# RobustFieldAutonomyLab/Distributional_RL_Navigation

Measured on AMD Instinct MI355X. Metric: env steps/sec (whole node) at 65 536 envs; IQN grad-steps/sec, higher is better.
Workload: dtype f32; 1 GPU; 65536 envs/GPU + IQN training (act K=32, 8 quantiles, replay 100000, batch 256, 1 grad step(s) every 4 vector steps); envs_per_gpu=65536, n_cores=8, n_obstacles=10, precision=f64, learner=independent, ranks_per_gpu=1, act_variant=2, taus=per_env, resets=under_next_act, launches_per_grad_step=1, ablation=False

## Files before the change

distributional_rl_navigation_amd/csrc/mn_capi.hip:

```cpp
#include <math.h>
#include <stdio.h>
#include <stdlib.h>
#include <string.h>

#include <string>
#include <vector>

#include "mn_internal.h"

struct mn_handle {
    MnArrays A;
    MnDev P;
    mn_params params;
    std::vector<void *> allocs;
    std::string err;
    int step_parity = 0;
    int last_parity = 0;
    uint32_t *seeds_dev = nullptr;
    uint32_t *mask_count = nullptr;
    int32_t *list_scratch = nullptr;
    double *peek_scratch = nullptr;
    double *obs64_buf = nullptr, *rew64_buf = nullptr;
    double *traj_trace = nullptr;
    int32_t traj_trace_steps = 0, traj_trace_sub = 0;
// ... 59 lines not shown
        snprintf(b, sizeof(b), "handle lives on HIP device %d but the calling thread's current device is %d", h->device, cur);
        return fail(h, MN_ERR_INVALID, b);
    }
    if (h->reset_pending) {
        if (hipEventSynchronize(h->ev_reset_end) != hipSuccess) return fail(h, MN_ERR_HIP, "waiting for the asynchronous reset failed");
        h->reset_pending = false;
    }
    if (h->reset_owed) {
        const hipStream_t s = h->owed_stream;
        settle_owed(h, s);
        if (hipStreamSynchronize(s) != hipSuccess) return fail(h, MN_ERR_HIP, "waiting for the owed reset failed");
    }
    return MN_OK;
}
static void join_reset(mn_handle *h, hipStream_t s) {
    if (!h) return;
    if (h->reset_owed) {
        int cur = -1;
        if (hipGetDevice(&cur) == hipSuccess && cur == h->device) settle_owed(h, s);
    }
    if (h->reset_pending) {
        if (hipStreamWaitEvent(s, h->ev_reset_end, 0) == hipSuccess) h->reset_pending = false;
    }
}
#define MN_ON_DEVICE(h) do { int _rc = on_device(h); if (_rc) return _rc; } while (0)

extern "C" int mn_default_params(mn_params *p) {
    if (!p) return MN_ERR_INVALID;
    memset(p, 0, sizeof(*p));
    p->width = 50; p->height = 50; p->core_r = 0.5; p->v_rel_max = 1.0; p->p = 0.8;
    p->v_range[0] = 5; p->v_range[1] = 10; p->obs_r_range[0] = 1; p->obs_r_range[1] = 3;
    p->clear_r = 10.0; p->goal_dis = 2.0; p->timestep_penalty = -1.0; p->collision_penalty = -50.0;
    p->goal_reward = 100.0; p->discount = 0.99; p->min_start_goal_dis = 25.0;
    p->init_theta = M_PI / 4; p->init_speed = 0.0;
    p->dt = 0.1; p->robot_r = 0.8; p->max_speed = 2.0;
    p->a[0] = -0.4; p->a[1] = 0.0; p->a[2] = 0.4;
    p->w[0] = -M_PI / 6; p->w[1] = 0.0; p->w[2] = M_PI / 6;
    p->sonar_range = 10.0; p->sonar_angle = 2 * M_PI / 3;
    p->num_cores = 8; p->num_obs = 5; p->reset_start_and_goal = 1; p->random_reset_state = 1;
    p->set_boundary = 0; p->max_episode_steps = 1000; p->N = 10; p->num_beams = MN_NUM_BEAMS;
    p->precision = MN_PRECISION_MIXED;
    return MN_OK;
}

static int derive(mn_handle *h, const mn_params &p) {
    const int32_t keep_skip = h->P.debug_skip;
    if (p.num_beams != MN_NUM_BEAMS) return fail(h, MN_ERR_INVALID, "num_beams must be 11");
    if (p.num_cores < 0 || p.num_cores > MN_MAX_CORES) return fail(h, MN_ERR_INVALID, "num_cores out of [0, 8]");
    if (p.num_obs < 0 || p.num_obs > MN_MAX_OBS) return fail(h, MN_ERR_INVALID, "num_obs out of [0, 10]");
    if (p.N < 1 || p.N > 1000) return fail(h, MN_ERR_INVALID, "robot N out of range");
    if (p.precision != MN_PRECISION_F64 && p.precision != MN_PRECISION_MIXED) return fail(h, MN_ERR_INVALID, "bad precision");
    if (p.step_lanes != 0 && p.step_lanes != 1 && p.step_lanes != 2 && p.step_lanes != 4 && p.step_lanes != 8) return fail(h, MN_ERR_INVALID, "step_lanes must be 0 (default), 1, 2, 4 or 8");
    if (p.rollout_lanes != 0 && p.rollout_lanes != 2 && p.rollout_lanes != 4 && p.rollout_lanes != 8 && p.rollout_lanes != 16) return fail(h, MN_ERR_INVALID, "rollout_lanes must be 0 (default), 2, 4, 8 or 16");
    MnDev &d = h->P;
    const int32_t keep_n = d.n_stages;
    d.width = p.width; d.height = p.height; d.core_r = p.core_r; d.v_rel_max = p.v_rel_max; d.p = p.p;
    d.v_lo = p.v_range[0]; d.v_span = p.v_range[1] - p.v_range[0];
    d.or_lo = p.obs_r_range[0]; d.or_span = p.obs_r_range[1] - p.obs_r_range[0];
    d.clear_r = p.clear_r; d.goal_dis = p.goal_dis;
    d.timestep_penalty = p.timestep_penalty; d.collision_penalty = p.collision_penalty; d.goal_reward = p.goal_reward;
    d.min_start_goal_dis = p.min_start_goal_dis; d.init_theta = p.init_theta; d.init_speed = p.init_speed;
    d.dt = p.dt; d.robot_r = p.robot_r; d.max_speed = p.max_speed;
    double amax = p.a[0];
    for (int i = 0; i < 3; ++i) {
        d.a[i] = p.a[i]; d.w[i] = p.w[i]; if (p.a[i] > amax) amax = p.a[i];
        d.rot_c[i] = cos(p.w[i] * p.dt); d.rot_s[i] = sin(p.w[i] * p.dt);
    }
    d.k_drag = amax / p.max_speed;
    d.sonar_range = p.sonar_range;
    const double phi = p.sonar_angle / (p.num_beams - 1);
    const double a0 = -p.sonar_angle / 2;
    for (int i = 0; i < MN_NUM_BEAMS; ++i) {
        d.beam_rel[i] = a0 + i * phi;
        d.beam_cos[i] = cos(d.beam_rel[i]);
        d.beam_sin[i] = sin(d.beam_rel[i]);
    }
    d.fan_sin = sin(p.sonar_angle / 2); d.fan_cos = cos(p.sonar_angle / 2);
    d.fan_filter = (p.sonar_angle / 2 < 0.49 * M_PI) ? 1 : 0;
    d.two_pi = 2 * M_PI;
    d.two_pi_r = 2 * M_PI * p.core_r;
    d.two_pi_vrel = 2 * M_PI * p.v_rel_max;
    d.inv_two_pi_vrel = 1.0 / d.two_pi_vrel;
    d.two_pi_r_r = 2 * M_PI * p.core_r * p.core_r;
    d.binom_q = exp(1.0 * log(1.0 - 0.5));
    d.sg_lo_x = 2.0; d.sg_span_x = (p.width - 2.0) - 2.0; d.sg_lo_y = 2.0; d.sg_span_y = (p.height - 2.0) - 2.0;
    d.c_span_x = p.width - 0.0; d.c_span_y = p.height - 0.0;
    d.o_lo = 5.0; d.o_span_x = (p.width - 5.0) - 5.0; d.o_span_y = (p.height - 5.0) - 5.0;
    d.num_cores = p.num_cores; d.num_obs = p.num_obs; d.reset_start_and_goal = p.reset_start_and_goal;
    d.random_reset_state = p.random_reset_state; d.set_boundary = p.set_boundary;
    d.max_episode_steps = p.max_episode_steps; d.N = p.N;
    d.n_stages = keep_n;
    d.debug_skip = keep_skip;
    h->params = p;
    return MN_OK;
}

template <typename T>
static int dev_alloc(mn_handle *h, T **out, size_t count, bool zero = true) {
    void *p = nullptr;
    hipError_t e = hipMalloc(&p, count * sizeof(T));
    if (e != hipSuccess) { h->err = std::string("hipMalloc failed: ") + hipGetErrorString(e); return MN_ERR_ALLOC; }
    if (zero) { e = hipMemset(p, 0, count * sizeof(T)); if (e != hipSuccess) { h->err = hipGetErrorString(e); return MN_ERR_HIP; } }
    h->allocs.push_back(p);
    *out = (T *)p;
    return MN_OK;
}

extern "C" int mn_destroy(mn_handle *h) {
    if (!h) return MN_ERR_INVALID;
    int cur = -1;
    const bool moved = hipGetDevice(&cur) == hipSuccess && h->device >= 0 && cur != h->device;
    if (moved) (void)hipSetDevice(h->device);
    if (h->reset_owed) { const hipStream_t s = h->owed_stream; settle_owed(h, s); (void)hipStreamSynchronize(s); }
    for (hipEvent_t e : h->ev) (void)hipEventDestroy(e);
    for (hipEvent_t e : h->ev_reset) (void)hipEventDestroy(e);
    if (h->side) { (void)hipStreamSynchronize(h->side); (void)hipStreamDestroy(h->side); }
    if (h->ev_stepped) (void)hipEventDestroy(h->ev_stepped);
    if (h->ev_reset_end) (void)hipEventDestroy(h->ev_reset_end);
    if (h->seen_host) (void)hipHostFree((void *)h->seen_host);
    for (void *p : h->allocs) (void)hipFree(p);
    if (moved) (void)hipSetDevice(cur);
    delete h;
    return MN_OK;
}

extern "C" int mn_create(int32_t n_envs, const mn_params *p, mn_handle **out) {
    if (!out || !p || n_envs <= 0) return fail(nullptr, MN_ERR_INVALID, "mn_create: bad arguments");
    int ndev = 0;
    if (hipGetDeviceCount(&ndev) != hipSuccess || ndev == 0) return fail(nullptr, MN_ERR_NO_DEVICE, "no HIP device visible");
    mn_handle *h = new mn_handle();
    if (hipGetDevice(&h->device) != hipSuccess) { delete h; return fail(nullptr, MN_ERR_HIP, "hipGetDevice failed"); }
    memset(&h->A, 0, sizeof(h->A));
    memset(&h->P, 0, sizeof(h->P));
    h->P.timestep_scale = 1.0;
    h->params.precision = p->precision;
    int rc = derive(h, *p);
    if (rc) { g_create_err = h->err; delete h; return rc; }
    MnArrays &A = h->A;
    A.n = n_envs;
    A.npad = (n_envs + MN_PAD - 1) / MN_PAD * MN_PAD;
    const size_t np = (size_t)A.npad;
#define ALLOC(field, count)                                    \
    if ((rc = dev_alloc(h, &A.field, (count))) != MN_OK) {      \
        g_create_err = h->err;                                 \
        mn_destroy(h);                                         \
        return rc;                                             \
    }
    ALLOC(x, np) ALLOC(y, np) ALLOC(theta, np) ALLOC(speed, np) ALLOC(vx, np) ALLOC(vy, np)
    ALLOC(start_x, np) ALLOC(start_y, np) ALLOC(goal_x, np) ALLOC(goal_y, np) ALLOC(init_theta, np) ALLOC(init_speed, np)
    ALLOC(ep_t, np) ALLOC(tot_t, np) ALLOC(counts, np)
    ALLOC(cx, np * MN_MAX_CORES) ALLOC(cy, np * MN_MAX_CORES) ALLOC(cg, np * MN_MAX_CORES)
    ALLOC(ox, np * MN_MAX_OBS) ALLOC(oy, np * MN_MAX_OBS) ALLOC(orad, np * MN_MAX_OBS)
    ALLOC(qcx, np * MN_MAX_CORES) ALLOC(qcy, np * MN_MAX_CORES) ALLOC(qcg, np * MN_MAX_CORES)
    ALLOC(qox, np * MN_MAX_OBS) ALLOC(qoy, np * MN_MAX_OBS) ALLOC(qor, np * MN_MAX_OBS)
    ALLOC(mt, np * 624) ALLOC(mt_pos, np)
    A.qcap = (int32_t)(((np >> 6) + MN_QSHARDS - 1) / MN_QSHARDS * 64);
    ALLOC(queue_count, 2 * MN_QWORDS) ALLOC(queue, (size_t)MN_QSHARDS * A.qcap)
#undef ALLOC
    if ((rc = dev_alloc(h, &h->seeds_dev, np)) || (rc = dev_alloc(h, &h->mask_count, 1)) ||
        (rc = dev_alloc(h, &h->list_scratch, np)) || (rc = dev_alloc(h, &h->peek_scratch, np))) {
        g_create_err = h->err; mn_destroy(h); return rc;
    }
    {
        std::vector<double> v(np);
        for (size_t i = 0; i < np; ++i) v[i] = 5.0;
        (void)hipMemcpy(A.start_x, v.data(), np * 8, hipMemcpyHostToDevice);
// ... 917 lines not shown
```

distributional_rl_navigation_amd/csrc/mn_internal.h:

```cpp
#pragma once
#include <hip/hip_runtime.h>
#include <stdint.h>

#include "marinenav_hip.h"

#define MN_WAVE 64
#define MN_PAD 256
#define MN_FIX_SCALE 16777216.0
#define MN_FIX_INV (1.0 / 16777216.0)
#define MN_TAB_ROWS (3 * MN_MAX_CORES + 3 * MN_MAX_OBS)

struct MnArrays {
    int32_t n, npad;
    double *x, *y, *theta, *speed, *vx, *vy;
    double *start_x, *start_y, *goal_x, *goal_y, *init_theta, *init_speed;
    int32_t *ep_t;
    int64_t *tot_t;
    int32_t *counts;
    double *cx, *cy, *cg;
    double *ox, *oy, *orad;
    int32_t *qcx, *qcy, *qox, *qoy;
    float *qcg, *qor;
    uint32_t *mt;
    int32_t *mt_pos;
    double *obs64;
    double *rew64;
    double *traj;
    int32_t traj_n;
    uint32_t *queue_count;
    int32_t *queue;
    int32_t qcap;
};
#define MN_QSHARDS 32
#define MN_QSTRIDE 32
#define MN_QWORDS (MN_QSHARDS * MN_QSTRIDE)

struct MnDev {
    double width, height, core_r, v_rel_max, p, v_lo, v_span, or_lo, or_span, clear_r, goal_dis;
    double timestep_penalty, collision_penalty, goal_reward;
    double min_start_goal_dis, init_theta, init_speed;
    double dt, robot_r, max_speed, k_drag, a[3], w[3];
    double sonar_range;
    double beam_rel[MN_NUM_BEAMS], beam_cos[MN_NUM_BEAMS], beam_sin[MN_NUM_BEAMS];
    double rot_c[3], rot_s[3];
    double fan_sin, fan_cos;
    int32_t fan_filter;
    double two_pi;
    double two_pi_r;
    double two_pi_vrel;
    double inv_two_pi_vrel;
    double two_pi_r_r;
    double binom_q;
    double sg_lo_x, sg_span_x, sg_lo_y, sg_span_y;
    double c_span_x, c_span_y;
    double o_lo, o_span_x, o_span_y;
    double timestep_scale;
    int32_t num_cores, num_obs, reset_start_and_goal, random_reset_state, set_boundary, max_episode_steps, N;
    int32_t n_stages;
    int32_t debug_skip;
    int64_t sched_t[MN_MAX_STAGES];
    int32_t sched_nc[MN_MAX_STAGES], sched_no[MN_MAX_STAGES];
    double sched_md[MN_MAX_STAGES];
};

struct MnRing {
    const float *prev_obs;
    float *states, *next_states;
    int64_t *actions;
    float *rewards, *dones;
    int64_t ptr, cap;
};

#define MN_STATE_MAGIC 0x54534e4du
#define MN_STATE_VERSION 1
#define MN_STATE_HEADER_BYTES 1024
#define MN_STATE_F64_ROWS (12 + 3 * MN_MAX_CORES + 3 * MN_MAX_OBS + 1)
#define MN_STATE_I32_ROWS (3 + 3 * MN_MAX_CORES + 3 * MN_MAX_OBS)
#define MN_STATE_MT_WORDS 624
struct MnStateHeader {
    uint32_t magic, version;
    int32_t n, precision;
    int64_t bytes;
    int32_t header_bytes, qcap;
    mn_params params;
    int32_t n_stages, pad0;
    double timestep_scale;
    int64_t sched_t[MN_MAX_STAGES];
    int32_t sched_nc[MN_MAX_STAGES], sched_no[MN_MAX_STAGES];
    double sched_md[MN_MAX_STAGES];
    int32_t step_parity, last_parity;
    uint32_t tick;
    int32_t under_act_max, owed_max_rows;
    uint32_t has_peak;
    uint32_t peak, seen;
};
static_assert(sizeof(MnStateHeader) <= MN_STATE_HEADER_BYTES, "MnStateHeader outgrew its slot");
static inline int64_t mn_state_layout_bytes(int64_t n, int64_t qcap) {
    return MN_STATE_HEADER_BYTES + n * MN_STATE_MT_WORDS * 4 + 2 * MN_QWORDS * 4 + MN_QSHARDS * qcap * 4 + MN_STATE_F64_ROWS * n * 8 + MN_STATE_I32_ROWS * n * 4;
}
void mn_launch_state(bool save, const MnArrays &A, const MnStateHeader &hdr, void *blob, uint32_t *peak_dev, uint32_t *seen_dev, uint32_t *ready, hipStream_t s);

void mn_launch_step(const MnArrays &A, const MnDev &P, int precision, int lanes, const int32_t *actions, float *obs,
                    float *reward, uint8_t *done, uint8_t *info, int parity, const MnRing *ring, hipStream_t s);
void mn_launch_rollout(const MnArrays &A, const MnDev &P, int precision, int lanes, int n_steps, const int32_t *actions_in,
                       uint64_t seed, uint64_t step0, uint64_t env0, float *obs_out, float *obs_trace, float *reward_trace,
                       uint8_t *done_trace, uint8_t *info_trace, int32_t *action_trace, hipStream_t s);
void mn_launch_random_actions(uint64_t seed, uint64_t step, uint64_t env0, int n, int32_t *out, hipStream_t s);
void mn_launch_rollout_policy(const MnArrays &A, const MnDev &P, int precision, int n_steps, int policy, float *obs_io, float *obs_trace,
                              float *reward_trace, uint8_t *done_trace, uint8_t *info_trace, int32_t *action_trace, double *traj_trace, hipStream_t s);
void mn_launch_planner_act(const float *obs, int n, int policy, const double *a, const double *w, int32_t *actions, hipStream_t s);
void mn_launch_rollout_iqn_rows(const MnArrays &A, const MnDev &P, int precision, int n_steps, const uint32_t *image, uint64_t *rng_state, float cvar,
                                int adaptive, const float *cvar_row, const uint8_t *adaptive_row, float *obs_io, float *obs_trace, float *reward_trace,
                                uint8_t *done_trace, uint8_t *info_trace, int32_t *action_trace, float *cvar_trace, float *q_trace, double *traj_trace,
                                uint32_t *words, int32_t *steps_run, hipStream_t s);
void mn_launch_rollout_iqn_eval(const MnArrays &A, const MnDev &P, int precision, int n_steps, const uint32_t *image, uint64_t *rng_state, float cvar,
                                int adaptive, const float *cvar_row, const uint8_t *adaptive_row, float *obs_io, float *obs_trace, float *reward_trace,
                                uint8_t *done_trace, uint8_t *info_trace, int32_t *action_trace, float *cvar_trace, float *q_trace, double *traj_trace,
                                float *quantiles_trace, float *taus_trace, uint32_t *words, int32_t *steps_run, hipStream_t s);
void mn_launch_rollout_iqn_groups(const MnArrays &A, const MnDev &P, int precision, int n_steps, const uint32_t *images, int64_t image_stride,
                                  int rows_per_group, uint64_t *rng_states, const float *cvar_row, const uint8_t *adaptive_row, float *obs_io,
                                  float *obs_trace, float *reward_trace, uint8_t *done_trace, uint8_t *info_trace, int32_t *action_trace, float *cvar_trace,
                                  float *q_trace, uint32_t *group_words, int32_t *steps_run, hipStream_t s);
int mn_iqn_rollout_image(mn_iqn_ctx *c, const float *const *weights, hipStream_t s, const uint32_t **image, uint32_t **words);
void mn_launch_dqn_pack(const float *const *weights, float *image_dev, hipStream_t s);
void mn_launch_rollout_dqn(const MnArrays &A, const MnDev &P, int precision, int n_steps, const float *image, float *obs_io, float *obs_trace,
                           float *reward_trace, uint8_t *done_trace, uint8_t *info_trace, int32_t *action_trace, float *q_trace, double *traj_trace, hipStream_t s);
void mn_launch_rollout_dqn_groups(const MnArrays &A, const MnDev &P, int precision, int n_steps, const float *images, int64_t image_stride, int n_groups,
                                  int rows_per_group, float *obs_io, float *obs_trace, float *reward_trace, uint8_t *done_trace, uint8_t *info_trace,
                                  int32_t *action_trace, float *q_trace, hipStream_t s);
void mn_launch_reset_under_act(const MnArrays &A, const MnDev &P, int precision, const uint32_t *count_dev, const int32_t *list_dev, float *obs,
                               uint32_t *ready, uint32_t tick, uint32_t *peak_dev, uint32_t *peak_host, hipStream_t s);
void mn_launch_reset(const MnArrays &A, const MnDev &P, int precision, const uint32_t *count_dev, uint32_t count_host,
                     const int32_t *list_dev, int mode, float *obs, hipStream_t s, uint32_t *peak_dev = nullptr, uint32_t *peak_host = nullptr, bool sharded = false);
#define MN_PREP_RESET_MIN_BLOCKS 256
// ... 39 lines not shown
```

distributional_rl_navigation_amd/csrc/mn_reset_body.h:

```cpp
#pragma once
#include "mn_device.h"

#ifdef MN_ABLATION
#define MN_RSKIP(bit) ((P.debug_skip & (bit)) != 0)
#else
#define MN_RSKIP(bit) false
#endif

#define MT_N 624
#define MT_M 397

__device__ __forceinline__ uint32_t mt_temper(uint32_t y) {
    y ^= (y >> 11);
    y ^= (y << 7) & 0x9d2c5680u;
    y ^= (y << 15) & 0xefc60000u;
    y ^= (y >> 18);
    return y;
}

__device__ __forceinline__ uint32_t mt_twist(uint32_t cur, uint32_t nxt, uint32_t far) {
    const uint32_t y = (cur & 0x80000000u) | (nxt & 0x7fffffffu);
    return far ^ (y >> 1) ^ ((y & 1u) ? 0x9908b0dfu : 0u);
}

// ... 377 lines not shown
                    }
                    for (int i = 0; i < no && valid; ++i) {
                        const double dx = W.ox[i] - x, dy = W.oy[i] - y;
                        valid = !dist_le(dx * dx + dy * dy, W.orad[i] + r);
                    }
                }
                int used = nb;
                for (;;) {
                    const unsigned long long m = __ballot(valid);
                    if (!m) break;
                    const int j = first_lane(m);
                    const double xj = bcast(x, j), yj = bcast(y, j), rj = bcast(r, j);
                    if (lane == j) { W.ox[no] = x; W.oy[no] = y; W.orad[no] = r; valid = false; }
                    else if (valid && lane > j) {
                        const double dx = xj - x, dy = yj - y;
                        valid = !dist_le(dx * dx + dy * dy, rj + r);
                    }
                    ++no;
                    if (no == want_o) { used = j + 1; break; }
                }
                __syncthreads();
                tried += used;
                rng.advance(6 * used);
                if (no == want_o || tried >= 500) break;
            }
        }

        if (P.random_reset_state) {
            rng.ensure(4, lane);
            double u[2];
            rng.template fetch<2>(0, u);
            th0 = 0.0 + (P.two_pi - 0.0) * u[0];
            sp0 = 0.0 + (P.max_speed - 0.0) * u[1];
            rng.advance(4);
        } else {
            th0 = P.init_theta; sp0 = P.init_speed;
        }

        __syncthreads();
        rng.store(A, e, lane, MN_RSKIP(512));
        if (lane < MN_MAX_CORES) {
            const bool v = lane < nc;
            A.cx[lane * np + e] = v ? W.cx[lane] : 0.0;
            A.cy[lane * np + e] = v ? W.cy[lane] : 0.0;
            A.cg[lane * np + e] = v ? W.cg[lane] : 0.0;
        }
        if (lane < MN_MAX_OBS) {
            const bool v = lane < no;
            A.ox[lane * np + e] = v ? W.ox[lane] : 0.0;
            A.oy[lane * np + e] = v ? W.oy[lane] : 0.0;
            A.orad[lane * np + e] = v ? W.orad[lane] : 0.0;
        }
        if (lane == 0) {
            A.mt_pos[e] = rng.c.pos;
            A.counts[e] = nc | (no << 8);
            A.start_x[e] = sx; A.start_y[e] = sy; A.goal_x[e] = gx; A.goal_y[e] = gy;
            A.init_theta[e] = th0; A.init_speed[e] = sp0;
        }
    } else {
        const int cnt = A.counts[e];
        nc = cnt & 0xff; no = (cnt >> 8) & 0xff;
        if (lane < nc) { W.cx[lane] = A.cx[lane * np + e]; W.cy[lane] = A.cy[lane * np + e]; W.cg[lane] = A.cg[lane * np + e]; }
        if (lane < no) { W.ox[lane] = A.ox[lane * np + e]; W.oy[lane] = A.oy[lane * np + e]; W.orad[lane] = A.orad[lane * np + e]; }
        sx = A.start_x[e]; sy = A.start_y[e]; gx = A.goal_x[e]; gy = A.goal_y[e];
        th0 = A.init_theta[e]; sp0 = A.init_speed[e];
    }
    __syncthreads();

    if (lane < MN_MAX_CORES) {
        const bool v = lane < nc;
        A.qcx[lane * np + e] = v ? __double2int_rn(W.cx[lane] * MN_FIX_SCALE) : 0;
        A.qcy[lane * np + e] = v ? __double2int_rn(W.cy[lane] * MN_FIX_SCALE) : 0;
        A.qcg[lane * np + e] = v ? (float)W.cg[lane] : 0.0f;
    }
    if (lane < MN_MAX_OBS) {
        const bool v = lane < no;
        A.qox[lane * np + e] = v ? __double2int_rn(W.ox[lane] * MN_FIX_SCALE) : 0;
        A.qoy[lane * np + e] = v ? __double2int_rn(W.oy[lane] * MN_FIX_SCALE) : 0;
        A.qor[lane * np + e] = v ? (float)W.orad[lane] : 0.0f;
    }

    double cvx = 0.0, cvy = 0.0;
    {
        const double i1 = 1.0 / P.two_pi_r_r, i2 = 1.0 / P.two_pi;
        for (int k = 0; k < nc; ++k) {
            double ux, uy;
            mn_core_velocity<double, true>(W.cx[k] - sx, W.cy[k] - sy, W.cg[k], i1, i2, ux, uy);
            cvx += ux; cvy += uy;
        }
    }
    double sn, cs;
    sincos(th0, &sn, &cs);
    const double velx = sp0 * cs + cvx, vely = sp0 * sn + cvy;

    if (lane < MN_NUM_BEAMS) {
        const double angle = th0 + P.beam_rel[lane];
        const bool up = fabs(angle - 0.5 * 3.141592653589793) < 1e-03;
        const bool down = fabs(angle - 3 * 3.141592653589793 / 2) < 1e-03;
        double bx = P.beam_cos[lane], by = P.beam_sin[lane];
        if (up || down) {
            const double sg = up ? 1.0 : -1.0;
            bx = sg * sn; by = sg * cs;
        }
        MnBeam<M> beam;
        beam.init();
        for (int k = 0; k < (MN_RSKIP(256) ? 0 : no); ++k) {
            const double mx = W.ox[k] - sx, my = W.oy[k] - sy;
            double tc, h2;
            mn_beam_geom(cs * mx + sn * my, -sn * mx + cs * my, W.orad[k] * W.orad[k], bx, by, tc, h2);
            beam.update(tc, h2, (M)P.sonar_range);
        }
        const double td = PARITY ? (double)beam.dist : beam.dist64();
        W.beam[lane][0] = beam.hit() ? td * bx : 0.0;
        W.beam[lane][1] = beam.hit() ? td * by : 0.0;
    }
    __syncthreads();
    if (lane < MN_OBS_DIM) {
        double v;
        const double gdx = gx - sx, gdy = gy - sy;
        if (lane == 0) v = cs * velx + sn * vely;
        else if (lane == 1) v = -sn * velx + cs * vely;
        else if (lane == 2) v = cs * gdx + sn * gdy;
        else if (lane == 3) v = -sn * gdx + cs * gdy;
        else v = W.beam[(lane - 4) >> 1][(lane - 4) & 1];
        if (obs_out) {
            if (ready) __hip_atomic_store(reinterpret_cast<uint32_t *>(obs_out) + (size_t)e * MN_OBS_DIM + lane, __float_as_uint((float)v), __ATOMIC_RELAXED, __HIP_MEMORY_SCOPE_AGENT);
            else obs_out[(size_t)e * MN_OBS_DIM + lane] = (float)v;
        }
        if (PARITY && A.obs64) A.obs64[(size_t)e * MN_OBS_DIM + lane] = v;
    }
    if (lane == 0) {
        A.x[e] = sx; A.y[e] = sy; A.theta[e] = th0; A.speed[e] = sp0;
        A.vx[e] = velx; A.vy[e] = vely;
        A.ep_t[e] = 0;
    }
    if (ready) {
        asm volatile("s_waitcnt vmcnt(0)" ::: "memory");
        if (lane == 0) __hip_atomic_store(ready + e, tick, __ATOMIC_RELAXED, __HIP_MEMORY_SCOPE_AGENT);
    }
}
```

distributional_rl_navigation_amd/csrc/mn_step.hip:

```cpp
#include "mn_step_body.h"

namespace {

template <typename M, bool PARITY, int L, bool APPEND>
__global__ __launch_bounds__(MN_STEP_BLOCK, 2) void mn_step_kernel(MnArrays A, MnDev P, const int32_t *__restrict__ actions,
                                                      float *__restrict__ obs_out, float *__restrict__ reward_out,
                                                      uint8_t *__restrict__ done_out, uint8_t *__restrict__ info_out,
                                                      int parity, MnRing R) {
    using Lane = MnLane<M, PARITY, L>;
    const int tid = blockIdx.x * blockDim.x + threadIdx.x;
    const int e = tid / L;
    const int q = tid % L;

    if (tid < MN_QSHARDS) A.queue_count[(parity ^ 1) * MN_QWORDS + tid * MN_QSTRIDE] = 0u;

    Lane ln;
    ln.load(A, e, q);
    const int action = ln.active ? actions[e] : 0;
    float2 prev_head[2], prev_beam[Lane::BPL];
    if constexpr (APPEND) {
        const float2 *prow = reinterpret_cast<const float2 *>(R.prev_obs + (size_t)(ln.active ? e : 0) * MN_OBS_DIM);
        prev_head[0] = prow[0]; prev_head[1] = prow[1];
#pragma unroll
        for (int j = 0; j < Lane::BPL; ++j) {
            const int b = q + L * j;
            prev_beam[j] = prow[2 + (b < MN_NUM_BEAMS ? b : MN_NUM_BEAMS - 1)];
        }
    }

    const MnStepOut o = ln.template step<APPEND>(A, P, action, obs_out + (size_t)e * MN_OBS_DIM,
                                                 (PARITY && A.obs64) ? A.obs64 + (size_t)e * MN_OBS_DIM : nullptr, R, prev_head, prev_beam);
    ln.store(A);
    if (ln.active && q == 0) {
        reward_out[e] = (float)o.reward;
        done_out[e] = (uint8_t)o.done;
        info_out[e] = (uint8_t)o.info;
    }
    {
        const bool mine = ln.active && o.done && q == 0;
        const unsigned long long m = __ballot(mine);
        if (m) {
            const int lane = threadIdx.x & (MN_WAVE - 1);
            const int leader = __ffsll((long long)m) - 1;
            const int sh = __shfl((e >> 6) & (MN_QSHARDS - 1), leader);
            unsigned base = 0;
            if (lane == leader) base = atomicAdd(&A.queue_count[parity * MN_QWORDS + sh * MN_QSTRIDE], (unsigned)__popcll(m));
            base = __shfl(base, leader);
            if (mine) A.queue[(size_t)sh * A.qcap + base + __popcll(m & ((1ull << lane) - 1ull))] = e;
        }
    }
}

template <typename M, bool PARITY, bool APPEND>
void launch_l(int lanes, const MnArrays &A, const MnDev &P, const int32_t *actions, float *obs, float *reward,
              uint8_t *done, uint8_t *info, int parity, const MnRing &R, hipStream_t s) {
    const dim3 block(MN_STEP_BLOCK);
#define MN_LAUNCH(LL)                                                                                              \
    hipLaunchKernelGGL((mn_step_kernel<M, PARITY, LL, APPEND>), dim3((unsigned)((size_t)A.npad * LL / MN_STEP_BLOCK)), block, 0, s, A, P, \
                       actions, obs, reward, done, info, parity, R)
    if (lanes == 0) lanes = A.n <= 131072 ? (APPEND ? 4 : 2) : 1;
    switch (lanes) {
        case 1: MN_LAUNCH(1); break;
        case 4: MN_LAUNCH(4); break;
        case 8: MN_LAUNCH(8); break;
        default: MN_LAUNCH(2); break;
    }
#undef MN_LAUNCH
}

}

void mn_launch_step(const MnArrays &A, const MnDev &P, int precision, int lanes, const int32_t *actions, float *obs,
                    float *reward, uint8_t *done, uint8_t *info, int parity, const MnRing *ring, hipStream_t s) {
    static const MnRing none = {};
    if (precision == MN_PRECISION_F64) {
        if (ring) launch_l<double, true, true>(lanes, A, P, actions, obs, reward, done, info, parity, *ring, s);
        else launch_l<double, true, false>(lanes, A, P, actions, obs, reward, done, info, parity, none, s);
    } else {
        if (ring) launch_l<float, false, true>(lanes, A, P, actions, obs, reward, done, info, parity, *ring, s);
        else launch_l<float, false, false>(lanes, A, P, actions, obs, reward, done, info, parity, none, s);
    }
}
```

distributional_rl_navigation_amd/csrc/mn_step_body.h:

```cpp

#pragma once
#include "mn_device.h"

#ifdef MN_ABLATION
#define MN_SKIP(bit) ((P.debug_skip & (bit)) != 0)
#else
#define MN_SKIP(bit) false
#endif
#if defined(MN_ABLATION) && defined(MN_PHASE_VAR)
#define MN_TICK_BEGIN() unsigned long long mn_tick_prev = __builtin_amdgcn_s_memtime()
#define MN_TICK(k) do { __builtin_amdgcn_sched_barrier(0); const unsigned long long t_ = __builtin_amdgcn_s_memtime(); \
        if (blockIdx.x == 0 && threadIdx.x == 0) MN_PHASE_VAR[k] += t_ - mn_tick_prev; mn_tick_prev = t_; __builtin_amdgcn_sched_barrier(0); } while (0)
#else
#define MN_TICK_BEGIN() do { } while (0)
#define MN_TICK(k) do { } while (0)
#endif

#define MN_REAL_BRANCH() asm volatile("" ::: "memory")

#ifndef MN_STEP_BLOCK
#define MN_STEP_BLOCK 64
#endif

template <int L>
__device__ __forceinline__ float group_sum(float v) {
    if (L >= 2) v += __builtin_bit_cast(float, __builtin_amdgcn_update_dpp(0, __builtin_bit_cast(int, v), 0xB1, 0xF, 0xF, true));
    if (L >= 4) v += __builtin_bit_cast(float, __builtin_amdgcn_update_dpp(0, __builtin_bit_cast(int, v), 0x4E, 0xF, 0xF, true));
    if (L >= 8) v += __builtin_bit_cast(float, __builtin_amdgcn_update_dpp(0, __builtin_bit_cast(int, v), 0x141, 0xF, 0xF, true));
    return v;
}

template <int CTRL>
__device__ __forceinline__ double dpp_get(double v) {
    const long long b = __builtin_bit_cast(long long, v);
    const int lo = __builtin_amdgcn_update_dpp(0, (int)(b & 0xffffffffll), CTRL, 0xF, 0xF, true);
    const int hi = __builtin_amdgcn_update_dpp(0, (int)(b >> 32), CTRL, 0xF, 0xF, true);
    return __builtin_bit_cast(double, ((long long)hi << 32) | (long long)(unsigned int)lo);
}
template <int L, int CTRL>
__device__ __forceinline__ double dpp_add(double v) {
    const long long b = __builtin_bit_cast(long long, v);
    const int lo = __builtin_amdgcn_update_dpp(0, (int)(b & 0xffffffffll), CTRL, 0xF, 0xF, true);
    const int hi = __builtin_amdgcn_update_dpp(0, (int)(b >> 32), CTRL, 0xF, 0xF, true);
    return v + __builtin_bit_cast(double, ((long long)hi << 32) | (long long)(unsigned int)lo);
}

template <int L>
__device__ __forceinline__ double group_sum(double v) {
    if (L >= 2) v = dpp_add<L, 0xB1>(v);
    if (L >= 4) v = dpp_add<L, 0x4E>(v);
    if (L >= 8) v = dpp_add<L, 0x141>(v);
    return v;
}

template <int CTRL>
__device__ __forceinline__ void nearest_step(double &d2, double &r2, int &k) {
    const double od2 = dpp_get<CTRL>(d2), or2 = dpp_get<CTRL>(r2);
    const int ok = __builtin_amdgcn_update_dpp(0, k, CTRL, 0xF, 0xF, true);
    const bool take = (od2 < d2) || (od2 == d2 && ok < k);
    d2 = take ? od2 : d2; r2 = take ? or2 : r2; k = take ? ok : k;
}
template <int L>
__device__ __forceinline__ void group_nearest(double &d2, double &r2, int &k) {
    if (L >= 2) nearest_step<0xB1>(d2, r2, k);
    if (L >= 4) nearest_step<0x4E>(d2, r2, k);
    if (L >= 8) nearest_step<0x141>(d2, r2, k);
    if (L >= 16) nearest_step<0x140>(d2, r2, k);
}

struct MnStepOut {
    double reward;
    int done, info;
};

template <typename M, bool PARITY, int L>
struct MnLane {
    static constexpr int CPL = L <= MN_MAX_CORES ? MN_MAX_CORES / L : 1;
    static constexpr int BPL = (MN_NUM_BEAMS + L - 1) / L;
    static constexpr int OPL = (MN_MAX_OBS + L - 1) / L;
    static_assert(MN_MAX_CORES % L == 0 || L == 16, "L must divide 8, or be 16");
    static_assert(MN_STEP_BLOCK == 64 && L <= 16, "a lane group lives inside one wavefront (and one DPP row); the work-list hand-off below relies on it");

    int e, q;
    bool active;
    double x, y, theta, speed, gx, gy;
    M velx, vely;
    double dis_c;
    bool dis_ok;
    int ep_t, nc, no;
    long long tot_t;
    double ccx[CPL], ccy[CPL];
    M cgs[CPL];
    double obx[OPL], oby[OPL], obr[OPL];

    __device__ __forceinline__ void load(const MnArrays &A, int env, int lane_in_group) {
        e = env; q = lane_in_group;
        active = e < A.n;
        dis_c = 0.0; dis_ok = false;
        const int np = A.npad;
        x = A.x[e]; y = A.y[e]; theta = A.theta[e]; speed = A.speed[e];
        velx = (M)A.vx[e]; vely = (M)A.vy[e];
        gx = A.goal_x[e]; gy = A.goal_y[e];
        const int cnt = A.counts[e];
        ep_t = A.ep_t[e];
        tot_t = A.tot_t[e];
        double ccg[CPL];
        if (PARITY) {
#pragma unroll
            for (int j = 0; j < CPL; ++j) {
                const int k = (q & (MN_MAX_CORES - 1)) * CPL + j;
                ccx[j] = A.cx[k * np + e]; ccy[j] = A.cy[k * np + e]; ccg[j] = A.cg[k * np + e];
            }
#pragma unroll
            for (int j = 0; j < OPL; ++j) {
                const int k = min(q + L * j, MN_MAX_OBS - 1);
                obx[j] = A.ox[k * np + e]; oby[j] = A.oy[k * np + e]; obr[j] = A.orad[k * np + e];
            }
        } else {
            int qx[CPL], qy[CPL], px[OPL], py[OPL];
            float qg[CPL], pr[OPL];
#pragma unroll
            for (int j = 0; j < CPL; ++j) {
                const int k = (q & (MN_MAX_CORES - 1)) * CPL + j;
                qx[j] = A.qcx[k * np + e]; qy[j] = A.qcy[k * np + e]; qg[j] = A.qcg[k * np + e];
            }
#pragma unroll
            for (int j = 0; j < OPL; ++j) {
                const int k = min(q + L * j, MN_MAX_OBS - 1);
                px[j] = A.qox[k * np + e]; py[j] = A.qoy[k * np + e]; pr[j] = A.qor[k * np + e];
            }
#pragma unroll
            for (int j = 0; j < CPL; ++j) {
                ccx[j] = (double)qx[j] * MN_FIX_INV; ccy[j] = (double)qy[j] * MN_FIX_INV; ccg[j] = (double)qg[j];
            }
#pragma unroll
            for (int j = 0; j < OPL; ++j) {
                obx[j] = (double)px[j] * MN_FIX_INV; oby[j] = (double)py[j] * MN_FIX_INV; obr[j] = (double)pr[j];
            }
        }
        nc = cnt & 0xff; no = (cnt >> 8) & 0xff;
#pragma unroll
        for (int j = 0; j < CPL; ++j) {
            const bool v = (q & (MN_MAX_CORES - 1)) * CPL + j < nc;
            ccx[j] = v ? ccx[j] : 1.0e6;
            ccy[j] = v ? ccy[j] : 1.0e6;
            cgs[j] = v ? (M)ccg[j] : M(0);
        }
#pragma unroll
        for (int j = 0; j < OPL; ++j) {
            const bool v = q + L * j < no;
            obx[j] = v ? obx[j] : 1.0e6;
            oby[j] = v ? oby[j] : 1.0e6;
            obr[j] = v ? obr[j] : 0.0;
        }
    }

    __device__ __forceinline__ void store(const MnArrays &A) const {
        if (active && q == 0) {
            A.x[e] = x; A.y[e] = y; A.theta[e] = theta; A.speed[e] = speed;
            A.vx[e] = (double)velx; A.vy[e] = (double)vely;
            A.ep_t[e] = ep_t;
            A.tot_t[e] = tot_t;
        }
    }

    template <bool APPEND>
    __device__ __forceinline__ MnStepOut step(const MnArrays &A, const MnDev &P, int action_raw, float *__restrict__ obs_row,
                                              double *__restrict__ obs_row64, const MnRing &R, const float2 *prev_head,
                                              const float2 *prev_beam, float *__restrict__ obs_row_b = nullptr) {
        MN_TICK_BEGIN();
        int action = action_raw < 0 ? 0 : (action_raw > 8 ? 8 : action_raw);

        const double dbx = gx - x, dby = gy - y;
        double dis_before = dis_c;
        if (__any(!dis_ok)) {
            MN_REAL_BRANCH();
            dis_before = sqrt(fma(dbx, dbx, dby * dby));
        }

        const int ai = action / 3, wi = action - 3 * ai;
        const double acc = ai == 0 ? P.a[0] : (ai == 1 ? P.a[1] : P.a[2]);
        const double wdt = (wi == 0 ? P.w[0] : (wi == 1 ? P.w[1] : P.w[2])) * P.dt;
        const double rot_c = wi == 0 ? P.rot_c[0] : (wi == 1 ? P.rot_c[1] : P.rot_c[2]);
        const double rot_s = wi == 0 ? P.rot_s[0] : (wi == 1 ? P.rot_s[1] : P.rot_s[2]);
        const double dt = P.dt, two_pi = P.two_pi;

        const double inv_two_pi_r2 = 1.0 / P.two_pi_r_r;
        const double inv_two_pi = 1.0 / P.two_pi;

        while (theta < 0.0) theta += two_pi;
        while (theta >= two_pi) theta -= two_pi;
        double sn = 0.0, cs = 1.0;
        if (!MN_SKIP(4)) sincos(theta, &sn, &cs);

        MN_TICK(0);
        const int nsub = MN_SKIP(1) ? 0 : P.N;
        if constexpr (!PARITY) {
            typedef float f2 __attribute__((ext_vector_type(2)));
            constexpr int NP = CPL >= 2 ? CPL / 2 : 1;
            const float dtf = (float)dt, i2p = (float)inv_two_pi, i2pr = (float)inv_two_pi_r2;
            f2 rdx[NP], rdy[NP], gsv[NP];
#pragma unroll
            for (int p_ = 0; p_ < NP; ++p_) {
                if constexpr (CPL >= 2) {
                    rdx[p_] = (f2){(float)(ccx[2 * p_] - x), (float)(ccx[2 * p_ + 1] - x)};
                    rdy[p_] = (f2){(float)(ccy[2 * p_] - y), (float)(ccy[2 * p_ + 1] - y)};
                    gsv[p_] = (f2){(float)cgs[2 * p_], (float)cgs[2 * p_ + 1]};
                } else {
                    rdx[p_] = (f2){(float)(ccx[0] - x), 1.0e6f};
                    rdy[p_] = (f2){(float)(ccy[0] - y), 1.0e6f};
                    gsv[p_] = (f2){(float)cgs[0], 0.f};
                }
            }
            for (int s = 0; s < nsub; ++s) {
                float hx[NP], hy[NP];
#pragma unroll
                for (int p_ = 0; p_ < NP; ++p_) {
                    const f2 d2 = __builtin_elementwise_fma(rdx[p_], rdx[p_], rdy[p_] * rdy[p_]);
                    f2 f = (f2){__builtin_amdgcn_rcpf(d2.x), __builtin_amdgcn_rcpf(d2.y)} * i2p;
                    f.x = f.x < i2pr ? f.x : i2pr;
                    f.y = f.y < i2pr ? f.y : i2pr;
                    f *= gsv[p_];
                    const f2 ux = -rdy[p_] * f, uy = rdx[p_] * f;
                    hx[p_] = CPL >= 2 ? ux.x + ux.y : ux.x;
                    hy[p_] = CPL >= 2 ? uy.x + uy.y : uy.x;
                }
                float sx_, sy_;
                if constexpr (NP == 4) { sx_ = (hx[0] + hx[1]) + (hx[2] + hx[3]); sy_ = (hy[0] + hy[1]) + (hy[2] + hy[3]); }
                else if constexpr (NP == 2) { sx_ = hx[0] + hx[1]; sy_ = hy[0] + hy[1]; }
                else { sx_ = hx[0]; sy_ = hy[0]; }
                const float cvx = group_sum<L>(sx_), cvy = group_sum<L>(sy_);
                velx = (float)(speed * cs) + cvx;
                vely = (float)(speed * sn) + cvy;
                x = fma((double)velx, dt, x);
                y = fma((double)vely, dt, y);
                const f2 nvx = (f2){-velx, -velx}, nvy = (f2){-vely, -vely}, dt2 = (f2){dtf, dtf};
#pragma unroll
                for (int p_ = 0; p_ < NP; ++p_) {
                    rdx[p_] = __builtin_elementwise_fma(nvx, dt2, rdx[p_]);
                    rdy[p_] = __builtin_elementwise_fma(nvy, dt2, rdy[p_]);
                }
                speed = fma(fma(-P.k_drag, speed, acc), dt, speed);
                speed = fmin(fmax(speed, 0.0), P.max_speed);
                const double c2 = fma(cs, rot_c, -(sn * rot_s));
                sn = fma(sn, rot_c, cs * rot_s);
                cs = c2;
            }
            theta = fma((double)nsub, wdt, theta);
            while (theta < 0.0) theta += two_pi;
            while (theta >= two_pi) theta -= two_pi;
        } else {
            for (int s = 0; s < nsub; ++s) {
                double ux[CPL], uy[CPL];
#pragma unroll
                for (int j = 0; j < CPL; ++j)
                    mn_core_velocity<double>(ccx[j] - x, ccy[j] - y, cgs[j], inv_two_pi_r2, inv_two_pi, ux[j], uy[j]);
                double sx_, sy_;
                if constexpr (CPL == 8) {
                    sx_ = ((ux[0] + ux[1]) + (ux[2] + ux[3])) + ((ux[4] + ux[5]) + (ux[6] + ux[7]));
                    sy_ = ((uy[0] + uy[1]) + (uy[2] + uy[3])) + ((uy[4] + uy[5]) + (uy[6] + uy[7]));
                } else if constexpr (CPL == 4) { sx_ = (ux[0] + ux[1]) + (ux[2] + ux[3]); sy_ = (uy[0] + uy[1]) + (uy[2] + uy[3]); }
                else if constexpr (CPL == 2) { sx_ = ux[0] + ux[1]; sy_ = uy[0] + uy[1]; }
                else { sx_ = ux[0]; sy_ = uy[0]; }
                const double cvx = group_sum<L>(sx_), cvy = group_sum<L>(sy_);
                velx = speed * cs + cvx;
                vely = speed * sn + cvy;
                x = fma(velx, dt, x);
                y = fma(vely, dt, y);
                if (A.traj && q == 0 && active && s < A.traj_n) {
                    A.traj[((size_t)e * A.traj_n + s) * 2] = x;
                    A.traj[((size_t)e * A.traj_n + s) * 2 + 1] = y;
                }
                speed = fma(fma(-P.k_drag, speed, acc), dt, speed);
                speed = speed < 0.0 ? 0.0 : (speed > P.max_speed ? P.max_speed : speed);
                theta += wdt;
                theta = theta < 0.0 ? theta + two_pi : theta;
                theta = theta >= two_pi ? theta - two_pi : theta;
                const double c2 = fma(cs, rot_c, -(sn * rot_s));
                sn = fma(sn, rot_c, cs * rot_s);
                cs = c2;
            }
        }

        MN_TICK(1);
        const double dax = gx - x, day = gy - y;
        const double dis_after = sqrt(fma(dax, dax, day * day));
        dis_c = dis_after; dis_ok = true;

        constexpr int NGRP = MN_STEP_BLOCK / L;
        __shared__ double lst_x[MN_MAX_OBS][NGRP], lst_y[MN_MAX_OBS][NGRP];
        __shared__ M lst_r[MN_MAX_OBS][NGRP];
        const int tl = threadIdx.x / L;
        const int gshift = (threadIdx.x & 63) & ~(L - 1);
        int nrel = 0;
        double best = 1e300, best_r = 0.0;
        int best_k = 1 << 20;
        const double reach0 = P.sonar_range + 0.05;
        if (!MN_SKIP(8))
#pragma unroll
        for (int j = 0; j < OPL; ++j) {
            const int k = q + L * j;
            const double mx = obx[j] - x, my = oby[j] - y;
            const double rx_ = fma(cs, mx, sn * my), ry_ = fma(cs, my, -(sn * mx));
            const double d2 = fma(mx, mx, my * my);
            const bool in = k < no;
            const bool nearer = in && (d2 < best);
            best = nearer ? d2 : best;
            best_r = nearer ? obr[j] : best_r;
            best_k = nearer ? k : best_k;
            const double r = obr[j];
            const double reach = reach0 + r;
            const bool rel = in && (d2 <= reach * reach) &&
                             (!P.fan_filter || (fma(P.fan_sin, rx_, -(P.fan_cos * fabs(ry_))) >= -fma(1.0e-3, reach, r + 0.05)));
            const unsigned gbits = (unsigned)(__ballot(rel) >> gshift) & ((1u << L) - 1u);
            const int pos = nrel + __popc(gbits & ((1u << q) - 1u));
            if (rel) { lst_x[pos][tl] = rx_; lst_y[pos][tl] = ry_; lst_r[pos][tl] = (M)r; }
            nrel += __popc(gbits);
        }
        group_nearest<L>(best, best_r, best_k);
        if (L > 1) __syncthreads();
        const M range = (M)P.sonar_range;
        const double half_pi = 0.5 * 3.141592653589793, three_half_pi = 3 * 3.141592653589793 / 2;
        M bxo[BPL], byo[BPL];
        double bdx[BPL], bdy[BPL];
        MnBeam<M> beam[BPL];
#pragma unroll
        for (int j = 0; j < BPL; ++j) {
            const int b = q + L * j;
            const int bb = b < MN_NUM_BEAMS ? b : MN_NUM_BEAMS - 1;
            const double angle = theta + P.beam_rel[bb];
            const bool up = fabs(angle - half_pi) < 1e-03;
            const bool down = fabs(angle - three_half_pi) < 1e-03;
            bdx[j] = P.beam_cos[bb]; bdy[j] = P.beam_sin[bb];
            if (up || down) {
                const double sg = up ? 1.0 : -1.0;
                bdx[j] = sg * sn; bdy[j] = sg * cs;
            }
            beam[j].init();
        }
        MN_TICK(2);
        if (!MN_SKIP(2))
        for (int s_ = 0; __any(s_ < nrel); ++s_) {
            const bool v = s_ < nrel;
            const double ox_ = lst_x[s_][tl], oy_ = lst_y[s_][tl];
            const double rr = (double)lst_r[s_][tl];
            const double r2o = v ? rr * rr : -1.0;
#pragma unroll
            for (int j = 0; j < BPL; ++j) {
                double tc, h2;
                mn_beam_geom(ox_, oy_, r2o, bdx[j], bdy[j], tc, h2);
                beam[j].update(tc, h2, range);
            }
        }
#pragma unroll
        for (int j = 0; j < BPL; ++j) {
            const bool hit = beam[j].hit();
            const double td = PARITY ? (double)beam[j].dist : beam[j].dist64();
            bxo[j] = hit ? (M)(td * bdx[j]) : M(0);
            byo[j] = hit ? (M)(td * bdy[j]) : M(0);
        }

        MN_TICK(3);
        double reward = P.timestep_penalty;
        reward += dis_before - dis_after;
        const double thr = best_r + P.robot_r, thr2 = thr * thr;
        bool near_enough = best <= thr2;
        if (__any(fabs(best - thr2) <= thr2 * 0x1p-48)) {
            MN_REAL_BRANCH();
            near_enough = sqrt(best) <= thr;
        }
        const bool collide = no > 0 && near_enough;
        const bool reach = dis_after <= P.goal_dis;
        const bool out = (x < 0.0 || x > P.width) || (y < 0.0 || y > P.height);
        int info = reach ? MN_INFO_REACH_GOAL : MN_INFO_NORMAL;
        info = collide ? MN_INFO_COLLISION : info;
        info = ep_t >= P.max_episode_steps ? MN_INFO_TOO_LONG : info;
        info = (P.set_boundary && out) ? MN_INFO_OUT_OF_BOUNDARY : info;
        const int done = info != MN_INFO_NORMAL;
        reward = info == MN_INFO_COLLISION ? reward + P.collision_penalty : (info == MN_INFO_REACH_GOAL ? reward + P.goal_reward : reward);
        ep_t += 1;
        tot_t += 1;

        MN_TICK(4);
        if (active) {
            long long slot = -1;
            if constexpr (APPEND) {
                const long long first = (long long)A.n > R.cap ? (long long)A.n - R.cap : 0;
                if (e >= first) { slot = R.ptr + (e - first); slot = slot >= R.cap ? slot - R.cap : slot; }
            }
            float2 *rs = APPEND && slot >= 0 ? reinterpret_cast<float2 *>(R.states + slot * MN_OBS_DIM) : nullptr;
            float2 *rn = APPEND && slot >= 0 ? reinterpret_cast<float2 *>(R.next_states + slot * MN_OBS_DIM) : nullptr;
            if (q == 0) {
                const M c = (M)cs, s_ = (M)sn;
                const M o0 = MnMath<M>::fma_(c, velx, s_ * vely), o1 = MnMath<M>::fma_(c, vely, -(s_ * velx));
                const M o2 = (M)fma(cs, dax, sn * day), o3 = (M)fma(cs, day, -(sn * dax));
                *reinterpret_cast<float2 *>(obs_row) = make_float2((float)o0, (float)o1);
                *reinterpret_cast<float2 *>(obs_row + 2) = make_float2((float)o2, (float)o3);
                if (obs_row_b) {
                    *reinterpret_cast<float2 *>(obs_row_b) = make_float2((float)o0, (float)o1);
                    *reinterpret_cast<float2 *>(obs_row_b + 2) = make_float2((float)o2, (float)o3);
                }
                if constexpr (APPEND) {
                    if (rs) {
                        rs[0] = prev_head[0]; rs[1] = prev_head[1];
                        rn[0] = make_float2((float)o0, (float)o1); rn[1] = make_float2((float)o2, (float)o3);
                        R.actions[slot] = (int64_t)action_raw;
                        R.rewards[slot] = (float)reward;
                        R.dones[slot] = done ? 1.0f : 0.0f;
                    }
                }
                if (PARITY && obs_row64) {
                    A.rew64[e] = reward;
                    obs_row64[0] = (double)o0; obs_row64[1] = (double)o1; obs_row64[2] = (double)o2; obs_row64[3] = (double)o3;
                }
            }
            if (!MN_SKIP(16))
// ... 20 lines not shown
```

Measured before the change: 996.7 million env steps/s.

## Split step-kernel loads into staged phases and broadcast beam tables via bpermute

Splits the per-env load into a head load, an early obstacle load and a deferred obstacle conversion, with scheduling barriers so the obstacle loads are issued before the action and previous-observation reads and stay in flight during the dynamics loop. Beam angle and direction tables are loaded once per wave lane and fetched through ds_bpermute instead of per-lane indexed constant loads. Action parameters are forced into scalar registers, and reciprocals are precomputed on the host. This aims to hide global-memory latency and cut scalar/vector load traffic, at the cost of more live registers and possible occupancy pressure.

```diff
diff --git a/distributional_rl_navigation_amd/csrc/mn_capi.hip b/distributional_rl_navigation_amd/csrc/mn_capi.hip
--- a/distributional_rl_navigation_amd/csrc/mn_capi.hip
+++ b/distributional_rl_navigation_amd/csrc/mn_capi.hip
@@ -165,6 +165,8 @@
     d.two_pi_vrel = 2 * M_PI * p.v_rel_max;
     d.inv_two_pi_vrel = 1.0 / d.two_pi_vrel;
     d.two_pi_r_r = 2 * M_PI * p.core_r * p.core_r;
+    d.inv_two_pi_r2 = 1.0 / d.two_pi_r_r;
+    d.inv_two_pi = 1.0 / d.two_pi;
     d.binom_q = exp(1.0 * log(1.0 - 0.5));
     d.sg_lo_x = 2.0; d.sg_span_x = (p.width - 2.0) - 2.0; d.sg_lo_y = 2.0; d.sg_span_y = (p.height - 2.0) - 2.0;
     d.c_span_x = p.width - 0.0; d.c_span_y = p.height - 0.0;
diff --git a/distributional_rl_navigation_amd/csrc/mn_internal.h b/distributional_rl_navigation_amd/csrc/mn_internal.h
--- a/distributional_rl_navigation_amd/csrc/mn_internal.h
+++ b/distributional_rl_navigation_amd/csrc/mn_internal.h
@@ -50,6 +50,7 @@
     double two_pi_vrel;
     double inv_two_pi_vrel;
     double two_pi_r_r;
+    double inv_two_pi_r2, inv_two_pi;
     double binom_q;
     double sg_lo_x, sg_span_x, sg_lo_y, sg_span_y;
     double c_span_x, c_span_y;
diff --git a/distributional_rl_navigation_amd/csrc/mn_reset_body.h b/distributional_rl_navigation_amd/csrc/mn_reset_body.h
--- a/distributional_rl_navigation_amd/csrc/mn_reset_body.h
+++ b/distributional_rl_navigation_amd/csrc/mn_reset_body.h
@@ -483,7 +483,7 @@
 
     double cvx = 0.0, cvy = 0.0;
     {
-        const double i1 = 1.0 / P.two_pi_r_r, i2 = 1.0 / P.two_pi;
+        const double i1 = P.inv_two_pi_r2, i2 = P.inv_two_pi;
         for (int k = 0; k < nc; ++k) {
             double ux, uy;
             mn_core_velocity<double, true>(W.cx[k] - sx, W.cy[k] - sy, W.cg[k], i1, i2, ux, uy);
diff --git a/distributional_rl_navigation_amd/csrc/mn_step.hip b/distributional_rl_navigation_amd/csrc/mn_step.hip
--- a/distributional_rl_navigation_amd/csrc/mn_step.hip
+++ b/distributional_rl_navigation_amd/csrc/mn_step.hip
@@ -15,8 +15,10 @@
     if (tid < MN_QSHARDS) A.queue_count[(parity ^ 1) * MN_QWORDS + tid * MN_QSTRIDE] = 0u;
 
     Lane ln;
-    ln.load(A, e, q);
+    ln.load_head(A, e, q);
     const int action = ln.active ? actions[e] : 0;
+    __builtin_amdgcn_sched_barrier(0);
+    ln.load_obstacles(A);
     float2 prev_head[2], prev_beam[Lane::BPL];
     if constexpr (APPEND) {
         const float2 *prow = reinterpret_cast<const float2 *>(R.prev_obs + (size_t)(ln.active ? e : 0) * MN_OBS_DIM);
@@ -27,8 +29,10 @@
             prev_beam[j] = prow[2 + (b < MN_NUM_BEAMS ? b : MN_NUM_BEAMS - 1)];
         }
     }
+    ln.load_tables(P);
+    __builtin_amdgcn_sched_barrier(0);
 
-    const MnStepOut o = ln.template step<APPEND>(A, P, action, obs_out + (size_t)e * MN_OBS_DIM,
+    const MnStepOut o = ln.template step<APPEND, true>(A, P, action, obs_out + (size_t)e * MN_OBS_DIM,
                                                  (PARITY && A.obs64) ? A.obs64 + (size_t)e * MN_OBS_DIM : nullptr, R, prev_head, prev_beam);
     ln.store(A);
     if (ln.active && q == 0) {
diff --git a/distributional_rl_navigation_amd/csrc/mn_step_body.h b/distributional_rl_navigation_amd/csrc/mn_step_body.h
--- a/distributional_rl_navigation_amd/csrc/mn_step_body.h
+++ b/distributional_rl_navigation_amd/csrc/mn_step_body.h
@@ -17,6 +17,7 @@
 #endif
 
 #define MN_REAL_BRANCH() asm volatile("" ::: "memory")
+#define MN_UNIFORM(v) asm("" : "+s"(v))
 
 #ifndef MN_STEP_BLOCK
 #define MN_STEP_BLOCK 64
@@ -93,6 +94,72 @@
     M cgs[CPL];
     double obx[OPL], oby[OPL], obr[OPL];
 
+    int opx[OPL], opy[OPL];
+    float opr[OPL];
+    double tab;
+
+    __device__ __forceinline__ void load_head(const MnArrays &A, int env, int lane_in_group) {
+        e = env; q = lane_in_group;
+        active = e < A.n;
+        dis_c = 0.0; dis_ok = false;
+        const int np = A.npad;
+        x = A.x[e]; y = A.y[e]; theta = A.theta[e]; speed = A.speed[e];
+        velx = (M)A.vx[e]; vely = (M)A.vy[e];
+        gx = A.goal_x[e]; gy = A.goal_y[e];
+        const int cnt = A.counts[e];
+        ep_t = A.ep_t[e];
+        tot_t = A.tot_t[e];
+        double ccg[CPL];
+        if (PARITY) {
+#pragma unroll
+            for (int j = 0; j < CPL; ++j) {
+                const int k = (q & (MN_MAX_CORES - 1)) * CPL + j;
+                ccx[j] = A.cx[k * np + e]; ccy[j] = A.cy[k * np + e]; ccg[j] = A.cg[k * np + e];
+            }
+        } else {
+            int qx[CPL], qy[CPL];
+            float qg[CPL];
+#pragma unroll
+            for (int j = 0; j < CPL; ++j) {
+                const int k = (q & (MN_MAX_CORES - 1)) * CPL + j;
+                qx[j] = A.qcx[k * np + e]; qy[j] = A.qcy[k * np + e]; qg[j] = A.qcg[k * np + e];
+            }
+#pragma unroll
+            for (int j = 0; j < CPL; ++j) {
+                ccx[j] = (double)qx[j] * MN_FIX_INV; ccy[j] = (double)qy[j] * MN_FIX_INV; ccg[j] = (double)qg[j];
+            }
+        }
+        nc = cnt & 0xff; no = (cnt >> 8) & 0xff;
+#pragma unroll
+        for (int j = 0; j < CPL; ++j) {
+            const bool v = (q & (MN_MAX_CORES - 1)) * CPL + j < nc;
+            ccx[j] = v ? ccx[j] : 1.0e6;
+            ccy[j] = v ? ccy[j] : 1.0e6;
+            cgs[j] = v ? (M)ccg[j] : M(0);
+        }
+    }
+
+    __device__ __forceinline__ void load_obstacles(const MnArrays &A) {
+        const int np = A.npad;
+#pragma unroll
+        for (int j = 0; j < OPL; ++j) {
+            const int k = min(q + L * j, MN_MAX_OBS - 1);
+            if (PARITY) { obx[j] = A.ox[k * np + e]; oby[j] = A.oy[k * np + e]; obr[j] = A.orad[k * np + e]; }
+            else { opx[j] = A.qox[k * np + e]; opy[j] = A.qoy[k * np + e]; opr[j] = A.qor[k * np + e]; }
+        }
+    }
+
+    __device__ __forceinline__ void finish_obstacles() {
+#pragma unroll
+        for (int j = 0; j < OPL; ++j) {
+            if (!PARITY) { obx[j] = (double)opx[j] * MN_FIX_INV; oby[j] = (double)opy[j] * MN_FIX_INV; obr[j] = (double)opr[j]; }
+            const bool v = q + L * j < no;
+            obx[j] = v ? obx[j] : 1.0e6;
+            oby[j] = v ? oby[j] : 1.0e6;
+            obr[j] = v ? obr[j] : 0.0;
+        }
+    }
+
     __device__ __forceinline__ void load(const MnArrays &A, int env, int lane_in_group) {
         e = env; q = lane_in_group;
         active = e < A.n;
@@ -155,6 +222,21 @@
         }
     }
 
+    static_assert(offsetof(MnDev, beam_cos) == offsetof(MnDev, beam_rel) + MN_NUM_BEAMS * sizeof(double) &&
+                  offsetof(MnDev, beam_sin) == offsetof(MnDev, beam_cos) + MN_NUM_BEAMS * sizeof(double) && 3 * MN_NUM_BEAMS <= MN_WAVE, "one bank: 33 consecutive doubles");
+    __device__ __forceinline__ void load_tables(const MnDev &P) {
+        if constexpr (L > 1) {
+            const int lane = threadIdx.x & (MN_WAVE - 1);
+            tab = (&P.beam_rel[0])[lane < 3 * MN_NUM_BEAMS ? lane : 3 * MN_NUM_BEAMS - 1];
+        }
+    }
+    __device__ __forceinline__ double table(int i) const {
+        const long long b = __builtin_bit_cast(long long, tab);
+        const int lo = __builtin_amdgcn_ds_bpermute(i << 2, (int)(b & 0xffffffffll));
+        const int hi = __builtin_amdgcn_ds_bpermute(i << 2, (int)(b >> 32));
+        return __builtin_bit_cast(double, ((long long)hi << 32) | (long long)(unsigned int)lo);
+    }
+
     __device__ __forceinline__ void store(const MnArrays &A) const {
         if (active && q == 0) {
             A.x[e] = x; A.y[e] = y; A.theta[e] = theta; A.speed[e] = speed;
@@ -164,7 +246,7 @@
         }
     }
 
-    template <bool APPEND>
+    template <bool APPEND, bool ONE_STEP = false>
     __device__ __forceinline__ MnStepOut step(const MnArrays &A, const MnDev &P, int action_raw, float *__restrict__ obs_row,
                                               double *__restrict__ obs_row64, const MnRing &R, const float2 *prev_head,
                                               const float2 *prev_beam, float *__restrict__ obs_row_b = nullptr) {
@@ -179,14 +261,26 @@
         }
 
         const int ai = action / 3, wi = action - 3 * ai;
-        const double acc = ai == 0 ? P.a[0] : (ai == 1 ? P.a[1] : P.a[2]);
-        const double wdt = (wi == 0 ? P.w[0] : (wi == 1 ? P.w[1] : P.w[2])) * P.dt;
-        const double rot_c = wi == 0 ? P.rot_c[0] : (wi == 1 ? P.rot_c[1] : P.rot_c[2]);
-        const double rot_s = wi == 0 ? P.rot_s[0] : (wi == 1 ? P.rot_s[1] : P.rot_s[2]);
+        double acc, wdt, rot_c, rot_s;
+        if constexpr (ONE_STEP) {
+            double a0 = P.a[0], a1 = P.a[1], a2 = P.a[2], w0 = P.w[0], w1 = P.w[1], w2 = P.w[2];
+            double rc0 = P.rot_c[0], rc1 = P.rot_c[1], rc2 = P.rot_c[2], rs0 = P.rot_s[0], rs1 = P.rot_s[1], rs2 = P.rot_s[2];
+            MN_UNIFORM(a0); MN_UNIFORM(a1); MN_UNIFORM(a2); MN_UNIFORM(w0); MN_UNIFORM(w1); MN_UNIFORM(w2);
+            MN_UNIFORM(rc0); MN_UNIFORM(rc1); MN_UNIFORM(rc2); MN_UNIFORM(rs0); MN_UNIFORM(rs1); MN_UNIFORM(rs2);
+            acc = ai == 0 ? a0 : (ai == 1 ? a1 : a2);
+            wdt = (wi == 0 ? w0 : (wi == 1 ? w1 : w2)) * P.dt;
+            rot_c = wi == 0 ? rc0 : (wi == 1 ? rc1 : rc2);
+            rot_s = wi == 0 ? rs0 : (wi == 1 ? rs1 : rs2);
+        } else {
+            acc = ai == 0 ? P.a[0] : (ai == 1 ? P.a[1] : P.a[2]);
+            wdt = (wi == 0 ? P.w[0] : (wi == 1 ? P.w[1] : P.w[2])) * P.dt;
+            rot_c = wi == 0 ? P.rot_c[0] : (wi == 1 ? P.rot_c[1] : P.rot_c[2]);
+            rot_s = wi == 0 ? P.rot_s[0] : (wi == 1 ? P.rot_s[1] : P.rot_s[2]);
+        }
         const double dt = P.dt, two_pi = P.two_pi;
 
-        const double inv_two_pi_r2 = 1.0 / P.two_pi_r_r;
-        const double inv_two_pi = 1.0 / P.two_pi;
+        const double inv_two_pi_r2 = P.inv_two_pi_r2;
+        const double inv_two_pi = P.inv_two_pi;
 
         while (theta < 0.0) theta += two_pi;
         while (theta >= two_pi) theta -= two_pi;
@@ -283,6 +377,7 @@
         }
 
         MN_TICK(1);
+        if constexpr (ONE_STEP) finish_obstacles();
         const double dax = gx - x, day = gy - y;
         const double dis_after = sqrt(fma(dax, dax, day * day));
         dis_c = dis_after; dis_ok = true;
@@ -328,10 +423,11 @@
         for (int j = 0; j < BPL; ++j) {
             const int b = q + L * j;
             const int bb = b < MN_NUM_BEAMS ? b : MN_NUM_BEAMS - 1;
-            const double angle = theta + P.beam_rel[bb];
+            const double angle = theta + (ONE_STEP && L > 1 ? table(bb) : P.beam_rel[bb]);
             const bool up = fabs(angle - half_pi) < 1e-03;
             const bool down = fabs(angle - three_half_pi) < 1e-03;
-            bdx[j] = P.beam_cos[bb]; bdy[j] = P.beam_sin[bb];
+            bdx[j] = ONE_STEP && L > 1 ? table(MN_NUM_BEAMS + bb) : P.beam_cos[bb];
+            bdy[j] = ONE_STEP && L > 1 ? table(2 * MN_NUM_BEAMS + bb) : P.beam_sin[bb];
             if (up || down) {
                 const double sg = up ? 1.0 : -1.0;
                 bdx[j] = sg * sn; bdy[j] = sg * cs;
```

Result: faster. 1.016 billion env steps/s, median of 6 (+1.9%).
